# zrudnick/bramble

Hardware: AMD Instinct MI355X
Metric: projected alignments/sec vs GENCODE-scale annotation (higher is better)
Workload: dtype u32; 1 GPU; device-resident (inputs already in HBM, packed rows left in HBM): 10M paired-end 2x100 short reads (name-collated, unstranded) vs GENCODE-shaped synthetic annotation (250836 transcripts, 1684128 transcript-exon rows, 25 refs); BASELINE.json configs[1]; group_lanes=8, seed=0xb4a3b1e

## Files before the change

### bramble_amd/csrc/abi.cpp

```cpp
#include <hip/hip_runtime.h>

#include <algorithm>
#include <atomic>
#include <cstdio>
#include <cstdlib>
#include <cstring>
#include <functional>
#include <string>
#include <thread>
#include <unordered_map>
#include <vector>

#include "ctx.h"
#include "primary_pick.h"

int check_device(int device) {
  int n = 0;
  hipError_t e = hipGetDeviceCount(&n);
  if (e != hipSuccess || n <= 0 || device >= n) return BR_ERR_NO_DEVICE;
  return BR_OK;
}

template <typename T>
static int upload(void **dst, const std::vector<T> &src, size_t &acc) {
// ... 350 lines not shown
  for (auto &S : c->stage) if (S.ready) (void)hipEventDestroy(S.ready);
  for (auto &S : c->in_slot) {
    if (S.ready) (void)hipEventDestroy(S.ready);
    if (S.rows_home) (void)hipEventDestroy(S.rows_home);
  }
  if (c->rows_busy) (void)hipEventDestroy(c->rows_busy);
  if (c->alt.busy) (void)hipEventDestroy(c->alt.busy);
  if (c->side2_stream) (void)hipStreamDestroy(c->side2_stream);
  if (c->side_stream) { (void)hipStreamDestroy(c->side_stream); for (auto &p : c->side_ev) for (auto &e : p) if (e) (void)hipEventDestroy(e); }
  if (c->run_stream) (void)hipStreamDestroy(c->run_stream);
  if (c->d2h_stream) (void)hipStreamDestroy(c->d2h_stream);
  if (c->copy_stream) (void)hipStreamDestroy(c->copy_stream);
  if (c->down_stream) (void)hipStreamDestroy(c->down_stream);
  for (int k = 0; k < 2; k++) if (c->ev_home[k]) (void)hipEventDestroy(c->ev_home[k]);
  delete c;
}

extern "C" int br_ctx_set_profiling(br_ctx *c, int enabled) {
  if (!c) return BR_ERR_INVALID_ARG;
  if (enabled && !c->profiling) for (int k = 0; k < BR_K_NUM; k++) { c->k_ms_sum[k] = 0; c->k_launches_sum[k] = 0; }
  c->profiling = enabled != 0;
  return BR_OK;
}
extern "C" int br_ctx_kernel_ms_sum(br_ctx *c, int which, double *ms, int64_t *launches) {
  if (!c || which < 0 || which >= BR_K_NUM) return BR_ERR_INVALID_ARG;
  if (ms) *ms = c->k_ms_sum[which];
  if (launches) *launches = c->k_launches_sum[which];
  return BR_OK;
}
extern "C" int br_ctx_set_param(br_ctx *c, const char *key, int64_t v) {
  if (!c || !key) return BR_ERR_INVALID_ARG;
  if (!strcmp(key, "group_lanes")) { if (v != 8 && v != 16 && v != 32 && v != 64) return BR_ERR_INVALID_ARG; c->group_lanes = (int)v; return BR_OK; }
  if (!strcmp(key, "direct_rows")) { c->direct_rows = v != 0; return BR_OK; }
  if (!strcmp(key, "small_batch")) { c->small_batch = v != 0; return BR_OK; }
  if (!strcmp(key, "speculate")) { c->speculate = v != 0; return BR_OK; }
  if (!strcmp(key, "speculate_n")) { if (v < 0) return BR_ERR_INVALID_ARG; c->speculate_n = v; return BR_OK; }
  if (!strcmp(key, "small_n")) { if (v < 0) return BR_ERR_INVALID_ARG; c->small_n = v; return BR_OK; }
  if (!strcmp(key, "deflate_dynamic")) { c->deflate_dynamic = v != 0; return BR_OK; }
  if (!strcmp(key, "bam_lanes")) { if (v != 0 && v != 4 && v != 8 && v != 16 && v != 32 && v != 64) return BR_ERR_INVALID_ARG; c->bam_lanes = (int)v; return BR_OK; }
  if (!strcmp(key, "ksw_fast")) { c->ksw_fast = v != 0; return BR_OK; }
  if (!strcmp(key, "ksw_tape_pct")) { if (v < 0 || v > 100) return BR_ERR_INVALID_ARG; c->ksw_tape_pct = (int)v; return BR_OK; }
  if (!strcmp(key, "ksw_tape_mb")) { if (v < 1) return BR_ERR_INVALID_ARG; c->ksw_tape_mb = v; return BR_OK; }
  if (!strcmp(key, "host_detail")) { c->host_detail = v != 0; return BR_OK; }
  if (!strcmp(key, "split_spoil")) { if (v < 0 || v > 1000000) return BR_ERR_INVALID_ARG; c->split_spoil = (int)v; return BR_OK; }
  if (!strcmp(key, "side_cap")) { if (v < 64) return BR_ERR_INVALID_ARG; c->d_side_cap = (uint64_t)v; return BR_OK; }
  if (!strcmp(key, "blocks_per_cu")) { if (v < 1 || v > 64) return BR_ERR_INVALID_ARG; c->blocks_per_cu = (int)v; return BR_OK; }
  return BR_ERR_INVALID_ARG;
}
extern "C" int br_ctx_kernel_ms(br_ctx *c, int which, double *ms, int32_t *launches) {
  if (!c || which < 0 || which >= BR_K_NUM) return BR_ERR_INVALID_ARG;
  if (ms) *ms = c->k_ms[which];
  if (launches) *launches = c->k_launches[which];
  return BR_OK;
}
extern "C" int br_ctx_ksw_diag(br_ctx *c, uint64_t out[16]) {
  if (!c || !out) return BR_ERR_INVALID_ARG;
  memcpy(out, c->ksw_diag, sizeof(c->ksw_diag));
  out[7] = (uint32_t)c->rb->ksw_left_after;
  return BR_OK;
}

extern "C" int br_ctx_rescue_stats(br_ctx *c, uint64_t out[4]) {
  if (!c || !out) return BR_ERR_INVALID_ARG;
  memcpy(out, c->rescue_stats, sizeof(c->rescue_stats));
  return BR_OK;
}
// ... 48 lines not shown
```

### bramble_amd/csrc/ctx.h

```cpp
#pragma once
#include <hip/hip_runtime.h>

#include <atomic>
#include <cassert>
#include <string>
#include <vector>

#include "../../include/bramble_amd.h"
#include "device_types.h"
#include "devmem.h"
#include "kernels.h"

using namespace br;

struct br_index {
  int device = -1;
  std::vector<std::string> names;
  std::vector<uint32_t> lengths;
  uint32_t n_refs = 0;
  bool has_seq = false;
  std::vector<uint32_t> slab_off, s_start, s_pmax, s_tid, tx_first, bin_off;
  std::vector<uint4> t_bin;
  std::vector<uint4> s_row, tx_ex;
  std::vector<uint8_t> seq_pool;
// ... 44 lines not shown
  struct StageSlot { DevBuf blob, off, len; hipEvent_t ready = nullptr; std::vector<uint64_t> h_off; int64_t n = 0; };
  StageSlot stage[3];
  hipStream_t copy_stream = nullptr;
  struct InSlot {
    DevBuf ref_id, ref_start, flags, xs, ts, cigar_off64, cigar, mate_ref, mate_start, name_off64, names, lqseq, seq_off64, seqs;
    DevBuf cigar_off, name_off, seq_off, mate_idx, group_off, seq_src, isnew, group_pre;
    hipEvent_t ready = nullptr, rows_home = nullptr;
    int64_t n = -1; uint64_t n_words = 0, n_name = 0, n_seq = 0; bool has_seq = false, staged = false, rows_pending = false;
    PinnedVec<uint4> h_a; PinnedVec<uint64_t> h_c, h_row_off; PinnedVec<uint32_t> h_pool; PinnedVec<uint4> h_x;
    PinnedVec<int32_t> h_mate, h_clip; PinnedVec<double> h_sim;
  };
  InSlot in_slot[2];
  hipStream_t run_stream = nullptr, d2h_stream = nullptr;
  hipEvent_t rows_busy = nullptr;
  bool rows_busy_set = false;
  struct RowSetAlt { DevBuf pk_a, pk_x, pk_sim, pk_clip, pk_ch, pool, row_off; hipEvent_t busy = nullptr; bool busy_set = false; } alt;
  int host_detail = 0;
  DevBuf z_slots, z_sizes, z_off, z_dense, z_dense_alt, z_tabs, z_tokens;
  DevBuf inf_out, inf_blocks, inf_tabs, inf_cnt; bool inf_tabs_ready = false;
  DevBuf sp_entry, sp_entry2, sp_exit, sp_nmap, sp_nunm, sp_ended, sp_redo, sp_pre, sp_small, sp_off, sp_len;
  DevBuf sf_names, sf_name_off, sf_len, sf_long, sf_small, sf_tmp, sf_text[2];
  int32_t sf_n_names = 0;
  int sf_which = 0;
  int z_dense_which = 0;
  hipStream_t down_stream = nullptr; hipEvent_t ev_home[2] = {nullptr, nullptr}; std::atomic<bool> home_pending[2] = {{false}, {false}};
  int deflate_dynamic = 1;
  int64_t speculate_n = 4194304;
  int speculate = 1;
  int64_t hist_n = 0; uint64_t hist[4] = {0, 0, 0, 0}; bool hist_simf = false;
  int small_batch = 1;
  int64_t small_n = 65536;
  DevBuf walk_list, pmask, pbit, pick;
  int direct_rows = 1;
  DevBuf d_fm, d_nkept, d_desc, d_hi0, d_clspos, d_rnd, d_side, d_sidectr;
  uint64_t d_side_cap = 0;
  int d_side_attempts = 0;
  bool last_direct = false;
  bool want_x = false;
  ProjectArgs dA{}; DirectArgs dD{}; int64_t d_kept = 0, d_simple = 0;
  DevBuf r_rec, pk_a, pk_c, pk_x, pk_sim, pk_clip;
  DevBuf pool, pool_sizes, pool_off, pk_ch;
  bool last_aux_cols = false;
  bool wide_valid = false;
  bool detail_valid = false;
  const int32_t *last_l_qseq = nullptr;
  int32_t last_long_reads = 0;
  int64_t last_n_pool = 0;
  bool z_tabs_ready = false;
  DevBuf p_ncig, p_name_len, p_isnew, p_group_pre, p_small, p_big, p_seq_len, p_ref_map;
  uint8_t *h_bam[2] = {nullptr, nullptr}; size_t h_bam_cap[2] = {0, 0}; int h_bam_next = 0;
  BigPinned h_bam_mem[2];
  int64_t last_n_rows = 0, last_n_aln = 0;
  br_device_bam last_bam{};
  br_device_rows last_rows{}; const uint32_t *last_group_off = nullptr; int64_t last_n_groups = 0; hipStream_t last_stream = nullptr;
  DevBuf fa_stats, fa_n_prob, fa_seq_bytes, fa_prob_off, fa_seqarena_off, fa_probs, fa_results, fa_seq_arena, fa_clip_ops,
      fa_ideal_cap, fa_scratch, fa_srcs, fa_want, b_seq_off, b_seqs, b_seq_src;
  DevBuf ksw_desc, ksw_dp, ksw_left, ksw_cnt, ksw_group, ksw_tape, ksw_raw;
  int ksw_fast = 1;
  hipStream_t side_stream = nullptr, side2_stream = nullptr;
  static constexpr int SIDE_EV = 8;
  hipEvent_t side_ev[SIDE_EV][2] = {}; int side_live = 0;
  uint32_t ksw_groups[KSW_N_BINS] = {0};
  int64_t ksw_tape_mb = 49152;
  int ksw_tape_pct = 100;
  uint64_t ksw_diag[16] = {0};
  DevBuf n_rows, row_off, aln_group;
// ... 92 lines not shown
```

### bramble_amd/csrc/direct_kernels.inc

```

#define WAVE_SYNC()                                                \
  do {                                                             \
    __builtin_amdgcn_fence(__ATOMIC_RELEASE, "workgroup");         \
    __builtin_amdgcn_wave_barrier();                               \
    __builtin_amdgcn_fence(__ATOMIC_ACQUIRE, "workgroup");         \
  } while (0)

__global__ void __launch_bounds__(256) k_name_seed(DirectArgs D) {
  const int64_t g = (int64_t)blockIdx.x * blockDim.x + threadIdx.x;
  if (g >= D.n_groups) return;
  const uint32_t a0 = D.group_off[g];
  const uint32_t no = D.name_off[a0];
  Mt64Lazy gen;
  gen.seed(hash_bytes(D.names + no, D.name_off[a0 + 1] - no));
  D.rnd0[g] = gen();
}
__device__ __forceinline__ uint32_t pick_from(uint64_t z0, const uint8_t *name, uint64_t len, uint32_t n) {
  uint64_t hi, lo;
  mul64wide(z0, (uint64_t)n, hi, lo);
  if (lo < (uint64_t)n) {
    const uint64_t thr = (0 - (uint64_t)n) % (uint64_t)n;
    if (lo < thr) return primary_pick(name, len, n);
  }
  return (uint32_t)hi;
// ... 3 lines not shown
#define PM_CAP_WIDE 8192
template <int CAP>
struct PmSh {
  uint32_t tid[CAP] __attribute__((aligned(16)));
  uint8_t bit[CAP], own4[CAP / 4];
  unsigned long long fmask[64];
  uint16_t poff[64];
  uint8_t pcnt[64], plane[64], same[64], one[64];
};
enum { PR_DEAD = 0, PR_SOLO = 1, PR_PAIR = 2 };

__device__ __forceinline__ uint32_t row_of_bit(uint32_t b, uint32_t lo0, uint32_t lo1, uint32_t n0) { return b < n0 ? lo0 + b : lo1 + (b - n0); }

__device__ __forceinline__ void stage_list(const uint32_t *__restrict__ s_tid, uint64_t mm, uint32_t lo0, uint32_t lo1, uint32_t n0,
                                           uint32_t *tid, uint8_t *bit, uint8_t *own4, uint32_t o, uint8_t owner) {
  while (mm) {
    uint32_t b[8], t[8]; bool ok[8];
#pragma unroll
    for (int u = 0; u < 8; u++) { ok[u] = mm != 0; b[u] = ok[u] ? (uint32_t)__builtin_ctzll(mm) : b[0]; mm &= mm - 1; }
#pragma unroll
    for (int u = 0; u < 8; u++) t[u] = s_tid[row_of_bit(b[u], lo0, lo1, n0)];
    *(uint4 *)&tid[o] = make_uint4(t[0], ok[1] ? t[1] : 0xffffffffu, ok[2] ? t[2] : 0xffffffffu, ok[3] ? t[3] : 0xffffffffu);
    *(uint32_t *)&bit[o] = b[0] | (b[1] << 8) | (b[2] << 16) | (b[3] << 24);
    own4[o >> 2] = owner;
    if (ok[4]) {
      *(uint4 *)&tid[o + 4] = make_uint4(t[4], ok[5] ? t[5] : 0xffffffffu, ok[6] ? t[6] : 0xffffffffu, ok[7] ? t[7] : 0xffffffffu);
      *(uint32_t *)&bit[o + 4] = b[4] | (b[5] << 8) | (b[6] << 16) | (b[7] << 24);
      own4[(o >> 2) + 1] = owner;
    }
    o += 8;
  }
}

template <int CAP>
__device__ __forceinline__ bool pair_window(const DirectArgs &D, PmSh<CAP> &S, int64_t w0, int lane) {
  const int64_t i64 = w0 + lane;
  const bool valid = i64 >= 0 && i64 < D.n_aln;
  const bool owner = valid && lane >= 1 && lane <= 62;
  const uint32_t i = (uint32_t)i64;
  uint32_t nm = 0, g = 0; uint64_t mk = 0; uint4 rg = make_uint4(0, 0, 0, 0); int32_t m = -1;
  if (valid) { nm = D.n_matches[i]; mk = D.mask[i]; rg = D.ranges[i]; m = D.mate_idx[i]; g = D.aln_group[i]; }
  const uint32_t n0 = rg.y - rg.x;
  const bool big = nm != 0 && (n0 + (rg.w - rg.z)) > 64u;
  const bool has_m = valid && m >= 0 && (int64_t)m < D.n_aln && (uint32_t)m != i;
  const int ml = has_m ? (int)((int64_t)m - w0) : -1;
  const bool m_in = ml >= 0 && ml < 64;
  const int src = m_in ? ml : lane;
  uint32_t g_m = __shfl(g, src), nm_m = __shfl(nm, src), big_m = __shfl((uint32_t)big, src);
  int32_t m_m = __shfl(m, src);
  uint64_t mk_p = 0; uint4 rg_p = make_uint4(0, 0, 0, 0);
  if (has_m && !m_in && owner) {
    g_m = D.aln_group[m]; m_m = D.mate_idx[m]; nm_m = D.n_matches[m]; mk_p = D.mask[m]; rg_p = D.ranges[m];
    big_m = (nm_m != 0 && ((rg_p.y - rg_p.x) + (rg_p.w - rg_p.z)) > 64u) ? 1u : 0u;
  }
  const bool mutual = has_m && g_m == g && m_m == (int32_t)i;
  const bool leader = !mutual || i < (uint32_t)m;
  int role = PR_DEAD;
  if (nm) { if (!mutual) role = PR_SOLO; else if (nm_m == 0) role = leader ? PR_SOLO : PR_DEAD; else role = PR_PAIR; }
  const bool defer = role != PR_DEAD && (big || (role == PR_PAIR && big_m));
  const uint32_t cnt = (uint32_t)__popcll(mk);
  if (owner && !defer && role != PR_PAIR) {
    const bool solo = role == PR_SOLO;
    D.fm[i] = solo ? make_uint2((uint32_t)mk, (uint32_t)(mk >> 32)) : make_uint2(0, 0);
    D.n_kept[i] = solo ? cnt : 0u; D.n_rows[i] = solo ? cnt : 0u; D.pflag[i] = 0;
  }
  const bool pair = role == PR_PAIR && !defer && (owner || m_in);
  if (!__ballot(pair && owner)) return true;
  const bool active = pair && (leader || !m_in);
  const uint32_t cnt4 = (cnt + 3u) & ~3u;
  const uint32_t ext = (active && !m_in) ? (uint32_t)__popcll(mk_p) : 0u;
  const uint32_t nA = active ? cnt4 : 0u, nP = (pair && !active ? cnt4 : 0u) + ((ext + 3u) & ~3u);
  uint32_t incA = nA, incP = nP;
#pragma unroll
  for (int d = 1; d < 64; d <<= 1) { const uint32_t ua = __shfl_up(incA, d), up = __shfl_up(incP, d); if (lane >= d) { incA += ua; incP += up; } }
  const uint32_t TA = __shfl(incA, 63), TP = __shfl(incP, 63);
  if (TA + TP > (uint32_t)CAP) return false;
  const uint32_t o_own = active ? incA - nA : TA + incP - nP;
  const uint32_t o_ext = TA + incP - nP;
  const uint32_t p_off = __shfl(o_own, src), p_cnt = __shfl(cnt, src);
  if (pair) {
    S.poff[lane] = (uint16_t)(m_in ? p_off : o_ext); S.pcnt[lane] = (uint8_t)(m_in ? p_cnt : ext);
    S.plane[lane] = (uint8_t)(m_in ? ml : 0xff); S.one[lane] = (cnt == 1u && (m_in ? p_cnt : ext) == 1u) ? 1 : 0;
  }
  S.fmask[lane] = 0; S.same[lane] = 0;
  if (pair) {
    stage_list(D.s_tid, mk, rg.x, rg.z, n0, S.tid, S.bit, S.own4, o_own, (uint8_t)lane);
    if (ext) stage_list(D.s_tid, mk_p, rg_p.x, rg_p.z, rg_p.y - rg_p.x, S.tid, S.bit, S.own4, o_ext, 0xff);
  }
  WAVE_SYNC();
  for (uint32_t e = lane; e < TA; e += 64) {
    const uint32_t t = S.tid[e];
    if (t == 0xffffffffu) continue;
    const uint32_t l = S.own4[e >> 2];
    const uint32_t p0 = S.poff[l], pe = p0 + S.pcnt[l];
    uint32_t y = 0xffffffffu;
    for (uint32_t x = p0; x < pe; x += 4) {
      const uint4 v = *(const uint4 *)&S.tid[x];
      y = v.x == t ? x : v.y == t ? x + 1 : v.z == t ? x + 2 : v.w == t ? x + 3 : y;
    }
    const bool found = y != 0xffffffffu;
    if (!found && !S.one[l]) continue;
    const uint32_t pl = S.plane[l];
    atomicOr(&S.fmask[l], 1ull << S.bit[e]);
    if (pl != 0xffu) atomicOr(&S.fmask[pl], 1ull << S.bit[found ? y : p0]);
    if (found) { S.same[l] = 1; if (pl != 0xffu) S.same[pl] = 1; }
  }
  WAVE_SYNC();
  if (pair && owner) {
    const uint64_t fmask = S.fmask[lane];
    const uint32_t nk = (uint32_t)__popcll(fmask);
    const bool paired = nk != 0;
    D.fm[i] = make_uint2((uint32_t)fmask, (uint32_t)(fmask >> 32));
    D.n_kept[i] = nk;
    D.n_rows[i] = leader ? 2u * nk : 0u;
    D.pflag[i] = (uint8_t)((paired ? PF_PAIRED : 0u) | ((paired && S.same[lane]) ? PF_SAME : 0u) | ((paired && !leader) ? PF_MATE : 0u));
  }
  return true;
}

__global__ void __launch_bounds__(256) k_pair_mask(DirectArgs D) {
  __shared__ PmSh<PM_CAP> sh_all[4];
  const int lane = threadIdx.x & 63, wv = threadIdx.x >> 6;
  const int64_t wi = (int64_t)blockIdx.x * 4 + wv;
  const int64_t w0 = wi * 62 - 1;
  if (w0 + 1 >= D.n_aln) return;
  if (!pair_window<PM_CAP>(D, sh_all[wv], w0, lane) && lane == 0) D.pm_list[atomicAdd(D.pm_n, 1u)] = (uint32_t)wi;
}
__global__ void __launch_bounds__(64) k_pair_mask_wide(DirectArgs D) {
  __shared__ PmSh<PM_CAP_WIDE> sh;
  const uint32_t n_work = *D.pm_n;
  for (uint32_t q = blockIdx.x; q < n_work; q += gridDim.x) {
    (void)pair_window<PM_CAP_WIDE>(D, sh, (int64_t)D.pm_list[q] * 62 - 1, (int)threadIdx.x);
    WAVE_SYNC();
  }
}

__device__ __forceinline__ void write_row(const DirectArgs &D, const uint4 E, uint32_t a, uint32_t c, uint32_t tid, uint32_t pos,
                                          uint32_t n_out, bool minus, uint64_t cig_ref, uint32_t junc, uint32_t refc) {
  const uint32_t fl = E.x & 0xffu, prim = E.x >> 8;
  const uint32_t stride = (fl & PF_PAIRED) ? 2u : 1u;
  const uint64_t r = (uint64_t)E.z + (uint64_t)stride * c;
  if (n_out > RM_NCIG) D.counters[3] = 1;
  const uint32_t meta = (n_out & RM_NCIG) | (minus ? RM_MINUS : 0u) | ((fl & PF_PAIRED) ? RM_PAIRED : 0u) | ((fl & PF_SAME) ? RM_SAME : 0u) |
                        ((fl & PF_MATE) ? 0u : RM_FIRST) | (prim == c + 1u ? RM_PRIMARY : 0u);
  typedef uint32_t nt4 __attribute__((ext_vector_type(4)));
  typedef uint32_t nt2 __attribute__((ext_vector_type(2)));
  const nt4 va = {tid, pos, meta, E.y};
  const nt2 vc = {(uint32_t)cig_ref, (uint32_t)(cig_ref >> 32)};
  __builtin_nontemporal_store(va, (nt4 *)(D.r_a + r));
  __builtin_nontemporal_store(vc, (nt2 *)(D.r_c + r));
  if (D.r_x) { const nt4 vx = {a, junc, refc, D.hi0[a] + stride * c}; __builtin_nontemporal_store(vx, (nt4 *)(D.r_x + r)); }
}


__device__ __forceinline__ unsigned long long side_need(uint32_t nb) {
  const unsigned long long x = ((unsigned long long)nb + 15ull) & ~15ull, k = (((unsigned long long)nb + 1ull) / 2ull + 15ull) & ~15ull;
  return x + k;
}
template <int EM>
__global__ void __launch_bounds__(64) k_big(ProjectArgs A, DirectArgs D) {
  __shared__ uint32_t sh_cig[EM ? 64 * LDS_SLOT : 1];
  __shared__ uint16_t sh_mops[EM ? 256 : 1];
  const int lane = threadIdx.x;
  if (EM) {
    for (int t = lane; t < 256; t += 64) sh_mops[t] = (uint16_t)((merge_action(t >> 4, t & 15u) << 8) | merge_ops(t >> 4, t & 15u));
// ... 496 lines not shown
  if (n_seg == 1) { p1.alive = true; p1.fwpos = h0.pos; p1.rcpos = h0.pos; p1.n_seg = 1; p1.n_gex = 1; p1.i_lastm = i0; p1.last_right_ins = h0.right_ins; p1.last_right_gap = h0.right_gap; }
  else if (!cfg.long_reads && !cfg.ignore_small_exons) {
    plain = true;
    p1.alive = true; p1.fwpos = h0.pos; p1.rcpos = h0.pos; p1.n_seg = n_seg; p1.n_gex = n_seg; p1.i_lastm = i0;
    p1.last_right_ins = 0; p1.last_right_gap = 0;
  }
  else p1 = walk_pass1(ix, cfg, rd, Ex, s == 1, sb, se, i0, make_uint4(gs, gend, pay.z, 0), make_uint2(r_a.z, r_b.w), q0, h0);
  const uint32_t ideal_cap = 4u * n_seg + 2u;
  const uint32_t cap = rd.n_real + 2u * ideal_cap;
  const uint64_t slot_off = D.cig_base[a] + (uint64_t)c * cap;
  uint32_t *slot = A.cig_arena + slot_off;
  uint32_t *lds = &sh_cig[(CLS == 1 ? 0 : threadIdx.x) * LDS_SLOT];
  const bool ideal_lds = ideal_cap <= LDS_IDEAL;
  uint32_t *ideal = ideal_lds ? lds : slot + rd.n_real + ideal_cap;
  Acc acc; IdealSink sk;
  sk.init(ideal);
  walk_pass2(ix, cfg, rd, Ex, s == 1, sb, se, i0, q0, make_uint4(gs, gend, pay.z, 0), make_uint2(r_a.z, r_b.w), h0, p1, acc, sk, no_clip(), no_clip());
  const uint32_t n_ideal = sk.finish();
  const bool out_lds = ideal_lds && (rd.n_real + n_ideal <= LDS_SLOT - LDS_IDEAL);
  uint32_t *outp = out_lds ? lds + LDS_IDEAL : slot;
  const uint32_t n_out = merge_cigars(rc, rd.n_real, ideal, n_ideal, outp, sh_mops);
  uint64_t cig_ref = slot_off;
  if (n_out <= 2) cig_ref = (uint64_t)(n_out > 0 ? outp[0] : 0u) | ((uint64_t)(n_out > 1 ? outp[1] : 0u) << 32);
  else if (out_lds) for (uint32_t q = 0; q < n_out; q++) slot[q] = outp[q];
  write_row(D, E, a, c, pay.x, (s == 0) ? p1.fwpos : (plain ? acc.last_pos : p1.rcpos), n_out, s == 1, cig_ref,
            (uint32_t)acc.junc_hits, (uint32_t)acc.ref_consumed);
}

static inline int grid_for_d(int64_t n, int per_block) { return (int)((n + per_block - 1) / per_block); }

void launch_name_seed(hipStream_t st, const DirectArgs &D) {
  if (D.n_groups > 0 && D.names) hipLaunchKernelGGL(k_name_seed, dim3(grid_for_d(D.n_groups, 256)), dim3(256), 0, st, D);
}
void launch_pair_mask(hipStream_t st, const DirectArgs &D, int wide_blocks) {
  if (D.n_aln <= 0) return;
  hipLaunchKernelGGL(k_pair_mask, dim3(grid_for_d(D.n_aln, 4 * 62)), dim3(256), 0, st, D);
  hipLaunchKernelGGL(k_pair_mask_wide, dim3(wide_blocks), dim3(64), 0, st, D);
}
void launch_big_collect(hipStream_t st, const ProjectArgs &A, const DirectArgs &D, int n_blocks) {
  if (D.n_aln > 0 && A.ix.n_rows != 0) hipLaunchKernelGGL((k_big<0>), dim3(n_blocks), dim3(64), 0, st, A, D);
}
void launch_pair_big(hipStream_t st, const DirectArgs &D, int n_blocks) {
  if (D.n_aln > 0) hipLaunchKernelGGL(k_pair_big, dim3(n_blocks), dim3(64), 0, st, D);
}
void launch_big_emit(hipStream_t st, const ProjectArgs &A, const DirectArgs &D, int n_blocks) {
  if (D.n_aln > 0 && A.ix.n_rows != 0) hipLaunchKernelGGL((k_big<1>), dim3(n_blocks), dim3(64), 0, st, A, D);
}
void launch_scan5(hipStream_t st, const DirectArgs &D, uint64_t *tile_sums, uint64_t *total_out5) {
  int64_t tiles = scan_tiles_for(D.n_aln);
  if (tiles < 1) tiles = 1;
  hipLaunchKernelGGL(k_scan5_tiles, dim3((unsigned)tiles), dim3(256), 0, st, D, tile_sums, tiles);
  hipLaunchKernelGGL(k_scan5_top, dim3(5), dim3(256), 0, st, tile_sums, tiles, total_out5);
  hipLaunchKernelGGL(k_scan5_apply, dim3((unsigned)tiles), dim3(256), 0, st, D, (const uint64_t *)tile_sums, tiles, (const uint64_t *)total_out5);
}
void launch_group_desc(hipStream_t st, const DirectArgs &D) {
  if (D.n_groups > 0) hipLaunchKernelGGL(k_group_desc, dim3(std::min(grid_for_d(D.n_groups, 256), 2048)), dim3(256), 0, st, D);
}
void launch_expand_rows(hipStream_t st, const DirectArgs &D) {
  if (D.n_aln > 0) hipLaunchKernelGGL(k_expand_rows, dim3(grid_for_d(D.n_aln, 256)), dim3(256), 0, st, D);
}
void launch_emit_rows(hipStream_t st, const ProjectArgs &A, const DirectArgs &D, int64_t n_kept, int64_t n_simple, int part) {
  if (A.n_aln <= 0 || n_kept <= 0) return;
  if (part == 1) { if (n_simple > 0) hipLaunchKernelGGL((k_emit_rows<1>), dim3(grid_for_d(n_simple, 256)), dim3(256), 0, st, A, D, (int64_t)0, n_simple); }
  else if (n_kept > n_simple) hipLaunchKernelGGL((k_emit_rows<2>), dim3(grid_for_d(n_kept - n_simple, 256)), dim3(256), 0, st, A, D, n_simple, n_kept);
}
```

### bramble_amd/csrc/kernels.h

```cpp
#pragma once
#include <hip/hip_runtime.h>
#include <stdint.h>

#include "device_types.h"
#include "ksw_types.h"
#include "scan_kernels.h"

namespace br {

enum {
  TOT_MATCHES = 0,
  TOT_ARENA = 1,
  TOT_SIMPLE = 2,
  TOT_ROWS = 3,
  TOT_RAW = 4,
  TOT_RESCUE_PROB = 5,
  TOT_RESCUE_SEQ = 6,
  TOT_WIDE_CIGAR = 7,
  TOT_SMALL_CNT = 8,
  TOT_PARSE_CIGAR = 12,
  TOT_PARSE_NAMES = 13,
  TOT_PARSE_GROUPS = 14,
  TOT_PARSE_SEQ = 15,
  TOT_BAM_LONG = 16,
// ... 166 lines not shown
  const uint32_t *n_matches;
  const uint64_t *mask;
  const uint4 *ranges;
  const uint32_t *fast_flag;
  const uint32_t *s_tid;
  const uint32_t *big_list; const uint32_t *n_big;
  uint2 *fm;
  uint32_t *n_kept;
  uint32_t *n_rows;
  uint8_t *pflag;
  uint2 *side;
  uint64_t side_cap;
  uint32_t *pm_list, *pm_n;
  unsigned long long *side_used;
  uint32_t *cls_pos;
  uint64_t *cig_base;
  uint64_t *row_off;
  const uint32_t *name_off; const uint8_t *names;
  uint64_t *rnd0;
  uint2 *gd;
  uint2 *dpos;
  uint32_t *hi0;
  uint64_t *counters;
  const uint64_t *tot;
  uint32_t *m_aln;
  uint64_t m_aln_cap;
  uint4 *r_a; uint2 *r_c;
  uint4 *r_x;
};
#define GD_SLOTS 16
#define GD_SLOT0 16
#define GD_SLOT_STRIDE 16
#define GD_COUNTER_WORDS (GD_SLOT0 + GD_SLOTS * GD_SLOT_STRIDE)
void launch_name_seed(hipStream_t st, const DirectArgs &D);
void launch_pair_mask(hipStream_t st, const DirectArgs &D, int wide_blocks);
void launch_big_collect(hipStream_t st, const ProjectArgs &A, const DirectArgs &D, int n_blocks);
void launch_pair_big(hipStream_t st, const DirectArgs &D, int n_blocks);
void launch_scan5(hipStream_t st, const DirectArgs &D, uint64_t *tile_sums, uint64_t *total_out5);
void launch_group_desc(hipStream_t st, const DirectArgs &D);
void launch_expand_rows(hipStream_t st, const DirectArgs &D);
void launch_emit_rows(hipStream_t st, const ProjectArgs &A, const DirectArgs &D, int64_t n_kept, int64_t n_simple, int part);
void launch_big_emit(hipStream_t st, const ProjectArgs &A, const DirectArgs &D, int n_blocks);

struct PoolArgs {
  int64_t n_rows;
  const uint4 *r_a; const uint2 *r_c;
  const uint32_t *arena;
  uint32_t *sizes;
  const uint64_t *off;
  uint2 *c_out;
  uint32_t *pool;
};

struct WideArgs {
  int64_t n_rows, n_aln;
  int32_t long_reads;
  const uint4 *r_a; const uint2 *r_c; const uint4 *r_x;
  const double *r_sim; const int32_t *r_clip;
  const uint32_t *pool;
  const uint32_t *aln_group;
  const int32_t *l_qseq;
  int32_t *w_input;
  uint32_t *w_nh, *w_hi, *w_mapq, *w_group;
  int32_t *w_mate_tid, *w_mate_pos, *w_isize;
  uint32_t *w_tid, *w_pos, *w_ncig;
  int8_t *w_strand;
  double *w_sim;
  int32_t *w_clip, *w_junc, *w_refc;
// ... 177 lines not shown
```

### bramble_amd/csrc/pipeline.cpp

```cpp
#include <algorithm>
#include <cstring>
#include <vector>

#include "ctx.h"

int ensure_side_stream(br_ctx *c) {
  if (c->side_stream) return BR_OK;
  HIPCHK(hipStreamCreateWithPriority(&c->side_stream, hipStreamNonBlocking, 0));
  for (auto &p : c->side_ev) for (auto &e : p) HIPCHK(hipEventCreateWithFlags(&e, hipEventDisableTiming));
  return BR_OK;
}

int run_ksw(br_ctx *c, hipStream_t st, const KswRun &R) {
  if (R.n_prob <= 0) return BR_OK;
  const uint64_t n_all = (uint64_t)R.n_prob;
  const uint64_t qmax = std::max<uint64_t>(R.qmax, 1), tmax = std::max<uint64_t>(R.tmax, 1);
  KswArgs K{};
  K.n_prob = R.n_prob; K.probs = R.probs; K.results = R.results; K.seq_arena = R.seq_arena; K.clip_ops = R.clip_ops;
  K.stats = R.stats;
  K.raw_out = R.raw_out; K.raw_n = R.raw_n; K.max_out = R.max_out; K.raw_cap = R.raw_cap;
  auto general = [&](uint64_t n_work, uint64_t q_hi, uint64_t t_hi, const uint32_t *list, const uint32_t *n_list) -> int {
    q_hi = std::max<uint64_t>(q_hi, 1); t_hi = std::max<uint64_t>(t_hi, 1);
    K.tmax = (uint32_t)t_hi;
    K.pmat_bytes = (size_t)(((q_hi + t_hi) * t_hi + 15) & ~15ull);
// ... 411 lines not shown
  D.gd = c->d_desc.as<uint2>(); D.dpos = c->d_desc.as<uint2>() + n; D.hi0 = c->d_hi0.as<uint32_t>(); D.counters = c->counters_d.as<uint64_t>(); D.tot = d_tot;

  SideWork seeds(c, st, ax2), pair_big(c, st, ax), group_desc(c, st, ax), big_emit(c, st, ax);
  HIPCHK(hipMemsetAsync(dz, 0, (GD_COUNTER_WORDS + 4) * 8, st));
  RC(pair_big.fork());
  RC(segment_stage(c, st, dc, b, pf));
  RC(pf.begin(BR_K_GROUP_IDS));
  launch_group_ids(st, ng, b->group_off, c->aln_group.as<uint32_t>());
  RC(pf.end());
  RC(count_pass(c, st, A, pf, true, true));
  if (c->rows_busy_set) { HIPCHK(hipStreamWaitEvent(st, c->rows_busy, 0)); }
  const int big_blocks = c->n_cu * 4;
  uint64_t kept = 0, arena = 0, n_simple = 0, n_rows = 0, n_raw = 0;
  bool expanded_ahead = false;
  if (have_names) {
    RC(seeds.fork());
    RC(pf.begin(BR_K_NAME_SEED, ax2));
    launch_name_seed(ax2, D);
    RC(pf.end());
    RC(seeds.done());
  }
  for (int attempt = 0;; attempt++) {
    if (attempt) {
      HIPCHK(hipMemsetAsync(dz, 0, (GD_COUNTER_WORDS + 2) * 8, st));
      HIPCHK(hipMemsetAsync(D.pm_n, 0, 4, st));
    }
    RC(pair_big.fork());
    RC(pf.begin(BR_K_PAIR_BIG, ax));
    launch_big_collect(ax, A, D, big_blocks);
    launch_pair_big(ax, D, big_blocks);
    RC(pf.end());
    RC(pair_big.done());
    RC(pf.begin(BR_K_PAIR_MASK));
    launch_pair_mask(st, D, c->n_cu * 2);
    RC(pf.end());
    RC(pair_big.join());
    RC(group_desc.fork());
    if (have_names) RC(seeds.join_on(ax));
    RC(pf.begin(BR_K_GROUP_DESC, ax));
    launch_group_desc(ax, D);
    RC(pf.end());
    RC(group_desc.done());
    RC(pf.begin(BR_K_SCAN));
    launch_scan5(st, D, c->tile_sums.as<uint64_t>(), d_tot);
    RC(pf.end());
    expanded_ahead = false;
    if (c->m_aln.cap >= 4) {
      D.m_aln = c->m_aln.as<uint32_t>(); D.m_aln_cap = c->m_aln.cap / 4;
      RC(pf.begin(BR_K_EXPAND_ROWS));
      launch_expand_rows(st, D);
      RC(pf.end());
      expanded_ahead = true;
    }
    HIPCHK(hipMemcpyAsync(rb->scan, d_tot, sizeof(rb->scan), hipMemcpyDeviceToHost, st));
    HIPCHK(hipMemcpyAsync(rb->side, dz + GD_COUNTER_WORDS, sizeof(rb->side), hipMemcpyDeviceToHost, st));
    HIPCHK(hipStreamSynchronize(st));
    c->d_side_attempts = attempt + 1;
    if (rb->side[1]) {
      if (attempt >= 3) return BR_ERR_CAPACITY;
      RC(group_desc.wait_host());
      c->d_side_cap = rb->side[0] + rb->side[0] / 4 + 4096;
      RC(c->d_side.ensure((size_t)c->d_side_cap * sizeof(uint2)));
      D.side = c->d_side.as<uint2>(); D.side_cap = c->d_side_cap;
      continue;
    }
    kept = rb->scan[TOT_MATCHES]; arena = rb->scan[TOT_ARENA]; n_simple = rb->scan[TOT_SIMPLE]; n_rows = rb->scan[TOT_ROWS]; n_raw = rb->scan[TOT_RAW];
    break;
// ... 320 lines not shown
    tmp.total_processed = (uint64_t)b->n_aln;
    if (tmp.row_off) { c->last_rows = tmp; c->last_group_off = b->group_off; c->last_n_groups = b->n_groups; }
  }
  DevBuf stats; RC(stats.ensure(8 * 8));
  HIPCHK(hipMemsetAsync(stats.p, 0, 8 * 8, st));
  StatsArgs T{};
  T.ix = c->ix->dev; T.n_aln = b->n_aln; T.ref_id = b->ref_id; T.cigar_off = b->cigar_off;
  T.seg = c->seg.as<uint2>(); T.head = c->head.as<uint4>(); T.head2 = c->head2.as<uint4>(); T.out = stats.as<uint64_t>();
  int64_t nm = (int64_t)c->counters[6];
  launch_stats(st, T, nm ? c->m_p.as<uint2>() : nullptr, c->match_off.as<uint32_t>(), c->n_matches.as<uint32_t>());
  uint64_t h[8];
  HIPCHK(hipMemcpyAsync(h, stats.p, 8 * 8, hipMemcpyDeviceToHost, st));
  HIPCHK(hipStreamSynchronize(st));
  uint64_t n = (uint64_t)b->n_aln;
  c->counters[3] = h[3]; c->counters[4] = h[4]; c->counters[5] = h[5]; c->counters[7] = h[7];
  c->counters[0] = 24ull * n + 4ull * h[3];
  c->counters[1] = h[1];
  c->counters[2] = 4ull * n + 24ull * (uint64_t)nm + 4ull * h[7];
  return BR_OK;
}

extern "C" int br_ctx_direct_diag(br_ctx *c, uint64_t out[8], uint8_t *pflags) {
  if (!c || !out || !c->last_direct) return BR_ERR_INVALID_ARG;
  HIPCHK(hipSetDevice(c->ix->device));
  const DirectArgs &D = c->dD;
  uint64_t used = 0;
  uint32_t nb[3] = {0, 0, 0};
  HIPCHK(hipDeviceSynchronize());
  HIPCHK(hipMemcpy(&used, D.side_used, 8, hipMemcpyDeviceToHost));
  HIPCHK(hipMemcpy(nb, D.n_big, 12, hipMemcpyDeviceToHost));
  if (pflags && D.n_aln > 0) HIPCHK(hipMemcpy(pflags, D.pflag, (size_t)D.n_aln, hipMemcpyDeviceToHost));
  memset(out, 0, 8 * sizeof(uint64_t));
  out[0] = nb[0]; out[1] = (uint64_t)c->d_side_attempts; out[2] = used; out[3] = D.side_cap; out[4] = nb[2];
  if (D.n_aln > 0) {
    const size_t n = (size_t)D.n_aln;
    std::vector<uint32_t> ff(n), nk(n);
    std::vector<uint4> hd(n);
    std::vector<uint8_t> pf(n);
    HIPCHK(hipMemcpy(ff.data(), D.fast_flag, n * 4, hipMemcpyDeviceToHost));
    HIPCHK(hipMemcpy(nk.data(), D.n_kept, n * 4, hipMemcpyDeviceToHost));
    HIPCHK(hipMemcpy(hd.data(), c->head.p, n * sizeof(uint4), hipMemcpyDeviceToHost));
    HIPCHK(hipMemcpy(pf.data(), D.pflag, n, hipMemcpyDeviceToHost));
    uint64_t light = 0;
    for (size_t a = 0; a < n; a++)
      if ((ff[a] >> 31) && hd[a].z == 2 && !(pf[a] & PF_BIG)) light += nk[a];
    out[5] = light;
  }
  return BR_OK;
}

extern "C" int br_project_batch_device(br_ctx *c, const br_config *cfg, const br_device_batch *b, void *stream,
                                       br_device_rows *out) {
  if (!c || !cfg || !b || !out) return BR_ERR_INVALID_ARG;
  return run_device(c, cfg, b, (hipStream_t)stream, out);
}

extern "C" int br_device_rows_expand(br_ctx *c, void *stream, br_device_wide_rows *out) {
  if (!c || !out) return BR_ERR_INVALID_ARG;
  return expand_rows(c, (hipStream_t)stream, out);
}
```

### bramble_amd/lib.py

```python
import ctypes as C
import os

import numpy as np

_HERE = os.path.dirname(os.path.abspath(__file__))
LIB_PATH = os.path.join(_HERE, "libbramble_amd.so")
_P = C.POINTER

K_SEGMENT, K_COUNT, K_EMIT, K_PAIR_COUNT, K_PAIR_EMIT, K_GATHER, K_SCAN, K_EMIT_AUX, K_KSW, K_BAM, K_PARSE, K_CODEC, K_EMIT_SIMPLE, K_PRIMARY, K_CIGAR_POOL, K_COUNT_WALK, K_EXPAND, K_GROUP_IDS, K_P1, K_P1_WALK, K_EMIT_WL, K_NAME_SEED, K_PAIR_MASK, K_PAIR_BIG, K_GROUP_DESC, K_EXPAND_ROWS, K_EMIT_ROWS_SIMPLE, K_EMIT_ROWS, K_BIG_EMIT, K_SAM_FORMAT, K_NUM = range(31)
KERNEL_NAMES = ["k_segment", "k_project<G,false,false,1>", "k_emit_dense<false,2>", "k_pair<false>", "k_pair<true>",
                "k_rows", "k_scan_*", "k_project<64,true>", "k_ksw", "k_bam_scan+k_bam_size+k_bam_encode",
                "k_rec_fields+k_group_off+k_rec_copy+k_mates+k_seq_*", "k_deflate_*+k_bgzf_compact",
                "k_emit_dense<false,1>", "k_primary", "(unused)", "k_project<G,false,false,2>", "k_expand", "k_group_ids",
                "(unused)", "(unused)", "(unused)", "k_name_seed", "k_pair_mask", "k_big<0>+k_pair_big", "k_group_desc",
                "k_expand_rows", "k_emit_rows<1>", "k_emit_rows<2>", "k_big<1>", "k_samfmt_*"]


class BrambleError(RuntimeError):
    pass


class BrExon(C.Structure):
    _fields_ = [("start", C.c_uint32), ("end", C.c_uint32)]

# ... 540 lines not shown

    @staticmethod
    def _device_batch_struct(dev_batch):
        db = BrDeviceBatch()
        db.n_aln = dev_batch["n_aln"]
        db.n_groups = dev_batch["n_groups"]
        for name in ("ref_id", "ref_start", "flags", "xs", "ts", "cigar_off", "cigar", "mate_idx", "group_off",
                     "l_qseq"):
            setattr(db, name, dev_batch[name].data_ptr())
        db.n_cigar_words = dev_batch["n_cigar_words"]
        db.max_n_cigar = dev_batch["max_n_cigar"]
        if dev_batch.get("seqs") is not None:
            db.seq_off = dev_batch["seq_off"].data_ptr()
            db.seqs = dev_batch["seqs"].data_ptr()
            db.seq_src = dev_batch["seq_src"].data_ptr()
            db.max_soft_clip = dev_batch["max_soft_clip"]
        if dev_batch.get("names") is not None:
            db.name_off = dev_batch["name_off"].data_ptr()
            db.names = dev_batch["names"].data_ptr()
        return db

    def collect_counters(self, dev_batch, stream=0):
        db = self._device_batch_struct(dev_batch)
        check(lib().br_ctx_collect_counters(self.h, C.byref(db), C.c_void_p(stream)), "br_ctx_collect_counters")
        out = (C.c_uint64 * 8)()
        check(lib().br_ctx_last_counters(self.h, out), "br_ctx_last_counters")
        keys = ("B_in", "B_idx", "B_out", "n_cigar", "read_exons", "overlap_hits", "matches", "out_cigar_words")
        return dict(zip(keys, [int(v) for v in out]))

    def direct_diag(self, n_aln=None):
        out = (C.c_uint64 * 8)()
        pf = np.zeros(n_aln, dtype=np.uint8) if n_aln is not None else None
        check(lib().br_ctx_direct_diag(self.h, out, pf.ctypes.data if pf is not None and n_aln else None), "br_ctx_direct_diag")
        d = dict(zip(("n_big", "side_attempts", "side_used", "side_cap", "pm_n", "light"), [int(v) for v in out[:6]]))
        if pf is not None:
            d["pflags"] = pf
        return d

    def project_bam_device(self, cfg, blob, rec_off, rec_len, ref_map, stream=0):
        recs = BrDeviceRecords()
        recs.blob = blob.data_ptr()
        recs.rec_off = rec_off.data_ptr()
        recs.n_aln = rec_len.numel()
        recs.rec_len = rec_len.data_ptr()
        rm = np.ascontiguousarray(ref_map, dtype=np.int32)
        rows, out = BrDeviceRows(), BrDeviceBam()
        check(lib().br_project_bam_device(self.h, C.byref(cfg), C.byref(recs), rm.ctypes.data, len(rm), C.c_void_p(stream),
                                          C.byref(rows), C.byref(out)), "br_project_bam_device")
        return rows, out

    def bgzf_deflate_device(self, src, stream=0):
        import torch
        from .device import _DevArray
        out, n = C.c_void_p(), C.c_uint64()
        check(lib().br_bgzf_deflate_device(self.h, C.c_void_p(src.data_ptr()), src.numel(), C.c_void_p(stream), C.byref(out),
                                           C.byref(n)), "br_bgzf_deflate_device")
        if n.value == 0:
            return torch.zeros(0, dtype=torch.uint8, device=src.device)
        return torch.as_tensor(_DevArray(out.value, n.value, "|u1"), device=src.device)

    def bgzf_inflate_device(self, src, blocks, stream=0):
        import torch
        from .device import _DevArray
        out, n = C.c_void_p(), C.c_uint64()
        blocks = np.ascontiguousarray(blocks, dtype=BGZF_BLOCK)
        L = lib()
        L.br_bgzf_inflate_device.argtypes = [C.c_void_p, C.c_void_p, C.c_uint64, C.c_void_p, C.c_int64, C.c_void_p, _P(C.c_void_p), _P(C.c_uint64)]
# ... 753 lines not shown
```

Before: 3.119 billion alignments/s.

## Add bitmask fast path for mate-pair transcript intersection in pair mask kernel

Adds a templated bitmask path to the pair-mask kernel. Each mate's candidate transcript IDs are folded into a 64-bit window mask, and the pair's shared transcripts come from an AND across lanes via shuffles. When both mates' transcript IDs fit in a 64-wide window, kept masks and flags are written directly, skipping the shared-memory list intersection. The path is enabled by default through a new param and adds a per-window atomic counter and a diagnostic readout. This costs extra ctz/gather work for every pair and more register pressure, while out-of-window pairs still fall back to the old path.

```diff
diff --git a/bramble_amd/csrc/abi.cpp b/bramble_amd/csrc/abi.cpp
--- a/bramble_amd/csrc/abi.cpp
+++ b/bramble_amd/csrc/abi.cpp
@@ -406,6 +406,7 @@
   if (!c || !key) return BR_ERR_INVALID_ARG;
   if (!strcmp(key, "group_lanes")) { if (v != 8 && v != 16 && v != 32 && v != 64) return BR_ERR_INVALID_ARG; c->group_lanes = (int)v; return BR_OK; }
   if (!strcmp(key, "direct_rows")) { c->direct_rows = v != 0; return BR_OK; }
+  if (!strcmp(key, "pair_bitmask")) { if (v != 0 && v != 1) return BR_ERR_INVALID_ARG; c->pair_bitmask = v != 0; return BR_OK; }
   if (!strcmp(key, "small_batch")) { c->small_batch = v != 0; return BR_OK; }
   if (!strcmp(key, "speculate")) { c->speculate = v != 0; return BR_OK; }
   if (!strcmp(key, "speculate_n")) { if (v < 0) return BR_ERR_INVALID_ARG; c->speculate_n = v; return BR_OK; }
diff --git a/bramble_amd/csrc/ctx.h b/bramble_amd/csrc/ctx.h
--- a/bramble_amd/csrc/ctx.h
+++ b/bramble_amd/csrc/ctx.h
@@ -100,6 +100,7 @@
   int64_t small_n = 65536;
   DevBuf walk_list, pmask, pbit, pick;
   int direct_rows = 1;
+  int pair_bitmask = 1;
   DevBuf d_fm, d_nkept, d_desc, d_hi0, d_clspos, d_rnd, d_side, d_sidectr;
   uint64_t d_side_cap = 0;
   int d_side_attempts = 0;
diff --git a/bramble_amd/csrc/direct_kernels.inc b/bramble_amd/csrc/direct_kernels.inc
--- a/bramble_amd/csrc/direct_kernels.inc
+++ b/bramble_amd/csrc/direct_kernels.inc
@@ -59,7 +59,34 @@
   }
 }
 
-template <int CAP>
+__device__ __forceinline__ void tids8(const uint32_t *__restrict__ s_tid, uint64_t &mm, uint32_t c0, uint32_t c1, uint32_t n0,
+                                      uint2 &pb, uint32_t (&t)[8]) {
+  uint32_t b[8];
+#pragma unroll
+  for (int u = 0; u < 8; u++) { b[u] = mm ? (uint32_t)__builtin_ctzll(mm) : b[0]; mm &= mm - 1; }
+#pragma unroll
+  for (int u = 0; u < 8; u++) t[u] = s_tid[b[u] + (b[u] < n0 ? c0 : c1)];
+  pb = make_uint2(b[0] | (b[1] << 8) | (b[2] << 16) | (b[3] << 24), b[4] | (b[5] << 8) | (b[6] << 16) | (b[7] << 24));
+}
+__device__ __forceinline__ void fold8(const uint32_t (&t)[8], uint32_t &lo, uint32_t &hi, uint64_t &tm) {
+  uint32_t rlo = t[0], rhi = t[0];
+#pragma unroll
+  for (int u = 1; u < 8; u++) { rlo = min(rlo, t[u]); rhi = max(rhi, t[u]); }
+  const uint32_t nlo = min(lo, rlo), sh = lo - nlo;
+  tm = sh > 63u ? 0ull : tm << sh;
+  lo = nlo; hi = max(hi, rhi);
+#pragma unroll
+  for (int u = 0; u < 8; u++) tm |= 1ull << ((t[u] - lo) & 63u);
+}
+
+__device__ __forceinline__ uint64_t keep8(uint2 pb, const uint32_t (&t)[8], uint64_t common, uint32_t base) {
+  uint64_t f = 0;
+#pragma unroll
+  for (int u = 0; u < 8; u++) f |= ((common >> ((t[u] - base) & 63u)) & 1ull) << (((u < 4 ? pb.x : pb.y) >> (8 * (u & 3))) & 63u);
+  return f;
+}
+
+template <int CAP, bool BM>
 __device__ __forceinline__ bool pair_window(const DirectArgs &D, PmSh<CAP> &S, int64_t w0, int lane) {
   const int64_t i64 = w0 + lane;
   const bool valid = i64 >= 0 && i64 < D.n_aln;
@@ -91,8 +118,51 @@
     D.fm[i] = solo ? make_uint2((uint32_t)mk, (uint32_t)(mk >> 32)) : make_uint2(0, 0);
     D.n_kept[i] = solo ? cnt : 0u; D.n_rows[i] = solo ? cnt : 0u; D.pflag[i] = 0;
   }
-  const bool pair = role == PR_PAIR && !defer && (owner || m_in);
+  bool pair = role == PR_PAIR && !defer && (owner || m_in);
   if (!__ballot(pair && owner)) return true;
+  uint64_t on_list = 0;
+  if (BM) {
+    const bool mp = pair && m_in;
+    uint32_t t0[8], t1[8], lo = 0xffffffffu, hi = 0;
+    uint2 pb0, pb1, pb;
+    const uint32_t c0 = rg.x, c1 = rg.z - n0;
+    uint64_t tm = 0, mm = mp ? mk : 0;
+    const bool any2 = __ballot(mp && cnt > 8u) != 0;
+    if (mm) tids8(D.s_tid, mm, c0, c1, n0, pb0, t0);
+    if (any2 && mm) tids8(D.s_tid, mm, c0, c1, n0, pb1, t1);
+    if (mp) fold8(t0, lo, hi, tm);
+    if (mp && cnt > 8u) fold8(t1, lo, hi, tm);
+    while (mm) { uint32_t t[8]; tids8(D.s_tid, mm, c0, c1, n0, pb, t); fold8(t, lo, hi, tm); }
+    const uint32_t lo_p = __shfl(lo, src), hi_p = __shfl(hi, src), cnt_p = __shfl(cnt, src);
+    const uint32_t base = min(lo, lo_p);
+    const bool fits = mp && max(hi, hi_p) - base <= 63u;
+    const uint64_t tmb = fits ? tm << (lo - base) : 0ull;
+    const uint64_t common = tmb & __shfl((unsigned long long)tmb, src);
+    if (fits) {
+      uint64_t fmask = mk;
+      if (common == 0) fmask = (cnt == 1u && cnt_p == 1u) ? mk : 0ull;
+      else if (common != tmb) {
+        fmask = keep8(pb0, t0, common, base);
+        if (cnt > 8u) fmask |= keep8(pb1, t1, common, base);
+        if (cnt > 16u) {
+          mm = mk;
+          for (int u = 0; u < 16; u++) mm &= mm - 1;
+          while (mm) { uint32_t t[8]; tids8(D.s_tid, mm, c0, c1, n0, pb, t); fmask |= keep8(pb, t, common, base); }
+        }
+      }
+      if (owner) {
+        const uint32_t nk = (uint32_t)__popcll(fmask);
+        const bool paired = nk != 0;
+        D.fm[i] = make_uint2((uint32_t)fmask, (uint32_t)(fmask >> 32));
+        D.n_kept[i] = nk;
+        D.n_rows[i] = leader ? 2u * nk : 0u;
+        D.pflag[i] = (uint8_t)((paired ? PF_PAIRED : 0u) | ((paired && common != 0) ? PF_SAME : 0u) | ((paired && !leader) ? PF_MATE : 0u));
+      }
+    }
+    pair = pair && !fits;
+    on_list = __ballot(pair && owner);
+    if (!on_list) return true;
+  }
   const bool active = pair && (leader || !m_in);
   const uint32_t cnt4 = (cnt + 3u) & ~3u;
   const uint32_t ext = (active && !m_in) ? (uint32_t)__popcll(mk_p) : 0u;
@@ -142,22 +212,27 @@
     D.n_rows[i] = leader ? 2u * nk : 0u;
     D.pflag[i] = (uint8_t)((paired ? PF_PAIRED : 0u) | ((paired && S.same[lane]) ? PF_SAME : 0u) | ((paired && !leader) ? PF_MATE : 0u));
   }
+  if (BM && lane == 0)
+    atomicAdd((unsigned long long *)&D.counters[GD_SLOT0 + (size_t)((uint64_t)(w0 + 1) / 62u & (GD_SLOTS - 1)) * GD_SLOT_STRIDE + PM_SLOT_WORD],
+              (unsigned long long)__popcll(on_list));
   return true;
 }
 
+template <bool BM>
 __global__ void __launch_bounds__(256) k_pair_mask(DirectArgs D) {
   __shared__ PmSh<PM_CAP> sh_all[4];
   const int lane = threadIdx.x & 63, wv = threadIdx.x >> 6;
   const int64_t wi = (int64_t)blockIdx.x * 4 + wv;
   const int64_t w0 = wi * 62 - 1;
   if (w0 + 1 >= D.n_aln) return;
-  if (!pair_window<PM_CAP>(D, sh_all[wv], w0, lane) && lane == 0) D.pm_list[atomicAdd(D.pm_n, 1u)] = (uint32_t)wi;
-}
+  if (!pair_window<PM_CAP, BM>(D, sh_all[wv], w0, lane) && lane == 0) D.pm_list[atomicAdd(D.pm_n, 1u)] = (uint32_t)wi;
+}
+template <bool BM>
 __global__ void __launch_bounds__(64) k_pair_mask_wide(DirectArgs D) {
   __shared__ PmSh<PM_CAP_WIDE> sh;
   const uint32_t n_work = *D.pm_n;
   for (uint32_t q = blockIdx.x; q < n_work; q += gridDim.x) {
-    (void)pair_window<PM_CAP_WIDE>(D, sh, (int64_t)D.pm_list[q] * 62 - 1, (int)threadIdx.x);
+    (void)pair_window<PM_CAP_WIDE, BM>(D, sh, (int64_t)D.pm_list[q] * 62 - 1, (int)threadIdx.x);
     WAVE_SYNC();
   }
 }
@@ -720,10 +795,14 @@
 void launch_name_seed(hipStream_t st, const DirectArgs &D) {
   if (D.n_groups > 0 && D.names) hipLaunchKernelGGL(k_name_seed, dim3(grid_for_d(D.n_groups, 256)), dim3(256), 0, st, D);
 }
-void launch_pair_mask(hipStream_t st, const DirectArgs &D, int wide_blocks) {
+template <bool BM>
+static void launch_pair_mask_t(hipStream_t st, const DirectArgs &D, int wide_blocks) {
+  hipLaunchKernelGGL((k_pair_mask<BM>), dim3(grid_for_d(D.n_aln, 4 * 62)), dim3(256), 0, st, D);
+  hipLaunchKernelGGL((k_pair_mask_wide<BM>), dim3(wide_blocks), dim3(64), 0, st, D);
+}
+void launch_pair_mask(hipStream_t st, const DirectArgs &D, int wide_blocks, bool bitmask) {
   if (D.n_aln <= 0) return;
-  hipLaunchKernelGGL(k_pair_mask, dim3(grid_for_d(D.n_aln, 4 * 62)), dim3(256), 0, st, D);
-  hipLaunchKernelGGL(k_pair_mask_wide, dim3(wide_blocks), dim3(64), 0, st, D);
+  if (bitmask) launch_pair_mask_t<true>(st, D, wide_blocks); else launch_pair_mask_t<false>(st, D, wide_blocks);
 }
 void launch_big_collect(hipStream_t st, const ProjectArgs &A, const DirectArgs &D, int n_blocks) {
   if (D.n_aln > 0 && A.ix.n_rows != 0) hipLaunchKernelGGL((k_big<0>), dim3(n_blocks), dim3(64), 0, st, A, D);
diff --git a/bramble_amd/csrc/kernels.h b/bramble_amd/csrc/kernels.h
--- a/bramble_amd/csrc/kernels.h
+++ b/bramble_amd/csrc/kernels.h
@@ -222,8 +222,9 @@
 #define GD_SLOT0 16
 #define GD_SLOT_STRIDE 16
 #define GD_COUNTER_WORDS (GD_SLOT0 + GD_SLOTS * GD_SLOT_STRIDE)
+#define PM_SLOT_WORD 2
 void launch_name_seed(hipStream_t st, const DirectArgs &D);
-void launch_pair_mask(hipStream_t st, const DirectArgs &D, int wide_blocks);
+void launch_pair_mask(hipStream_t st, const DirectArgs &D, int wide_blocks, bool bitmask);
 void launch_big_collect(hipStream_t st, const ProjectArgs &A, const DirectArgs &D, int n_blocks);
 void launch_pair_big(hipStream_t st, const DirectArgs &D, int n_blocks);
 void launch_scan5(hipStream_t st, const DirectArgs &D, uint64_t *tile_sums, uint64_t *total_out5);
diff --git a/bramble_amd/csrc/pipeline.cpp b/bramble_amd/csrc/pipeline.cpp
--- a/bramble_amd/csrc/pipeline.cpp
+++ b/bramble_amd/csrc/pipeline.cpp
@@ -467,7 +467,7 @@
     RC(pf.end());
     RC(pair_big.done());
     RC(pf.begin(BR_K_PAIR_MASK));
-    launch_pair_mask(st, D, c->n_cu * 2);
+    launch_pair_mask(st, D, c->n_cu * 2, c->pair_bitmask);
     RC(pf.end());
     RC(pair_big.join());
     RC(group_desc.fork());
@@ -854,6 +854,9 @@
   if (pflags && D.n_aln > 0) HIPCHK(hipMemcpy(pflags, D.pflag, (size_t)D.n_aln, hipMemcpyDeviceToHost));
   memset(out, 0, 8 * sizeof(uint64_t));
   out[0] = nb[0]; out[1] = (uint64_t)c->d_side_attempts; out[2] = used; out[3] = D.side_cap; out[4] = nb[2];
+  uint64_t slots[GD_COUNTER_WORDS];
+  HIPCHK(hipMemcpy(slots, D.counters, sizeof(slots), hipMemcpyDeviceToHost));
+  for (int k = 0; k < GD_SLOTS; k++) out[6] += slots[GD_SLOT0 + k * GD_SLOT_STRIDE + PM_SLOT_WORD];
   if (D.n_aln > 0) {
     const size_t n = (size_t)D.n_aln;
     std::vector<uint32_t> ff(n), nk(n);
diff --git a/bramble_amd/lib.py b/bramble_amd/lib.py
--- a/bramble_amd/lib.py
+++ b/bramble_amd/lib.py
@@ -596,7 +596,7 @@
         out = (C.c_uint64 * 8)()
         pf = np.zeros(n_aln, dtype=np.uint8) if n_aln is not None else None
         check(lib().br_ctx_direct_diag(self.h, out, pf.ctypes.data if pf is not None and n_aln else None), "br_ctx_direct_diag")
-        d = dict(zip(("n_big", "side_attempts", "side_used", "side_cap", "pm_n", "light"), [int(v) for v in out[:6]]))
+        d = dict(zip(("n_big", "side_attempts", "side_used", "side_cap", "pm_n", "light", "pm_list"), [int(v) for v in out[:7]]))
         if pf is not None:
             d["pflags"] = pf
         return d
```

After: 3.175 billion alignments/s, median of 6. +1.8%, better.
